# NorESMhub/BLOM

Hardware: AMD Instinct MI355X
Metric: simulated-days/sec (higher is better)
Workload: dtype f64; 1 GPU; channel 208x512x53 as 1 tile(s) of 208x512x53 along i, 1 tile per GPU, isopyc_bulkml/remap/geopotential/uc/enscon, ntr=3 (TKE, length-scale slot, ideal age: the reference default build), baclin=900s batrop=18s lstep=50; config 2's step (phy/mod_blom_step.F90:96-253: init_fluxes, tmsmt1, cmnfld2, difest_isobml [the whole routine: diffusivities estimated every step (NorESM defaults incl. rhsctp; the; physics=full, forcing=default, spinup_steps=0

## Files before the change

blom_amd/csrc/api.hip:

```cpp
#include "../../include/blomgpu.h"
#include "blomgpu_internal.h"
#include "pow_libm.h"
#include "sin_libm.h"
#include "atan2_libm.h"
#include <algorithm>
#include <cstring>
#include <string_view>

static thread_local std::string g_err;

int ctx_fail(blomgpu_ctx *c, const std::string &msg) {
  if (c) c->err = msg;
  g_err = msg;
  return 1;
}

void ctx_drop_graphs(blomgpu_ctx *c) {
  for (auto &g : c->step_graph)
    if (g) { (void)hipGraphExecDestroy(g); g = nullptr; }
  c->steps_warm = 0;
}

void ctx_sync_view(blomgpu_ctx *c) {
  if (!c->dirty) return;
// ... 401 lines not shown
  if (c->bt_flags) (void)hipFree(c->bt_flags);
  ale_free(c);
  dia_free(c);
  cesm_free(c);
  ben02_free(c);
  stepend_free(c);
  budget_free(c);
  if (c->ale_plevel) (void)hipFree(c->ale_plevel);
  if (c->arc_strip) (void)hipFree(c->arc_strip);
  if (c->xcsum_buf) (void)hipFree(c->xcsum_buf);
  if (c->xstream) (void)hipStreamDestroy(c->xstream);
  if (c->ev_fork) (void)hipEventDestroy(c->ev_fork);
  if (c->ev_join) (void)hipEventDestroy(c->ev_join);
  if (!c->stream_borrowed) (void)hipStreamDestroy(c->stream);
  delete c;
  return 0;
}

int blomgpu_sync(blomgpu_ctx *c) {
  HIPCHK(c, hipStreamSynchronize(c->stream));
  if (c->side) HIPCHK(c, hipStreamSynchronize(c->side));
  return 0;
}

int blomgpu_set_real(blomgpu_ctx *c, const char *name, double v) { return set_number(c, "blomgpu_set_real", name, 1u << O_REAL, v); }
int blomgpu_set_int(blomgpu_ctx *c, const char *name, int v) { return set_number(c, "blomgpu_set_int", name, 1u << O_INT | 1u << O_BOOL, v); }

int blomgpu_set_str(blomgpu_ctx *c, const char *name, const char *val) {
  const Opt *o = nullptr;
  const int rc = opt_lookup(c, "blomgpu_set_str", name, 1u << O_STR, &o);
  if (c) c->dirty = true;
  if (rc) return rc;
  if (!val) return ctx_fail(c, "blomgpu_set_str: null argument");
  const std::string v(val);
  if (!o->words[0].word) { *o->at(c).s = v; return 0; }
  for (const auto &w : o->words)
    if (w.word && v == w.word) {
      if (o->at) o->at(c).put(w.code);
      if (o->at && o->at(c).i == &c->swamth) c->swa_ready = false;
      return o->flags & ALE_RESET ? ale_reset(c) : 0;
    }
  return ctx_fail(c, o->refuse + v + " is unsupported!");
}

int blomgpu_get_real(blomgpu_ctx *c, const char *name, double *v) {
  const std::string s(name);
  if (const Opt *o = find_opt(s, 1u << O_REAL))
    if (o->flags & READABLE) { *v = *o->at(c).d; return 0; }
  if (s == "barotp_block_mode") { *v = bt_block_mode(c); return 0; }
  if (s == "barotp_shape") { *v = bt_shape_code(c); return 0; }
  if (s == "graph_steps") { *v = c->graph_steps; return 0; }
  if (s == "graph_failures") { *v = c->graph_failures; return 0; }
  if (s == "flux_diag_steps_skipped") { *v = (double)c->flux_diag_skipped; return 0; }
  if (s == "thermf_cesm_launches") { *v = (double)c->cesm_launches; return 0; }
  if (s == "thermf_ben02_launches") { *v = c->ben02_declared ? (double)c->cesm_launches : 0.; return 0; }
  if (c->step_time) {
    if (s == "xmi") { *v = c->xmi; return 0; }
    if (s == "nday_of_year") { *v = c->nday_of_year; return 0; }
    if (s.size() == 4 && s[0] == 'l' && s[1] >= '1' && s[1] <= '5' && s.compare(2, 2, "mi") == 0) { *v = c->lmi[s[1] - '1']; return 0; }
  }
  if (s == "sflxc") {
    if (!frc_declared(c)) return ctx_fail(c, "blomgpu_get_real: sflxc exists once blomgpu_inifrc_cesm has been called");
    double sum = 0.;
    HIPCHK(c, hipMemcpyAsync(&sum, c->cesm_sums, sizeof(double), hipMemcpyDeviceToHost, c->stream));
    HIPCHK(c, hipStreamSynchronize(c->stream));
    *v = sum / c->area;
    return 0;
  }
  if (s == "mxlayr_maxitr_entrain" || s == "mxlayr_maxitr_detrain") {
    *v = 0.;
    if (!c->err_dev) return 0;
    const int w = s == "mxlayr_maxitr_detrain" ? 5 : 6;
    int n = 0;
    HIPCHK(c, hipStreamSynchronize(c->stream));
    HIPCHK(c, hipMemcpy(&n, c->err_dev + w, sizeof(int), hipMemcpyDeviceToHost));
    HIPCHK(c, hipMemset(c->err_dev + w, 0, sizeof(int)));
    *v = n;
    return 0;
  }
  return ctx_fail(c, "blomgpu_get_real: unknown option " + s);
}

int blomgpu_option_name(int index, char *buf, int cap, int *kind) {
  if (index < 0 || index >= (int)(sizeof(g_opts) / sizeof(g_opts[0])) || !buf || cap < 2) return 1;
  snprintf(buf, cap, "%s", g_opts[index].name);
  if (kind) *kind = g_opts[index].kind;
  return 0;
}

int blomgpu_field_info(blomgpu_ctx *c, const char *name, int *nlev, int *is_int) {
  auto it = c->real_ids.find(name);
  if (it != c->real_ids.end()) {
    *nlev = ctx_real_nlev(c, it->second);
    if (std::string(name) == "trc" || std::string(name) == "trcold")
      *nlev = c->h.ntr * (std::string(name) == "trc" ? 2 : 1) * c->h.kk;
    *is_int = 0;
    return 0;
  }
  auto jt = c->int_ids.find(name);
  if (jt != c->int_ids.end()) { *nlev = c->nlev_int[jt->second]; *is_int = 1; return 0; }
  return ctx_fail(c, std::string("unknown field ") + name);
}

static int real_levels(blomgpu_ctx *c, const char *who, const char *name, int lev0, int nlev, double **ptr) {
  if (!c || !name) return ctx_fail(c, std::string(who) + ": null argument");
  auto it = c->real_ids.find(name);
// ... 472 lines not shown
    leave.failed = false;
  }
  if (!ale && (c->cmnfld1 || c->full_physics))
    if (int rc = stage(S_cmnfld1)) return rc;
  if (dia_active(c))
    if (int rc = st_diaacc(ALL6)) return rc;
  if (c->sprfac)
    if (int rc = st_fwbbal(c)) return rc;
  if (int rc = st_budget_output_instep(c)) return rc;
  if (c->chkvar) {
    c->seq.defer_checks = true;
    const int rc = st_chkvar(c, nn);
    c->seq.defer_checks = false;
    return rc;
  }
  return 0;
}
#undef ALL6
#undef STAGE_ARGS

int blomgpu_step(blomgpu_ctx *c, int *nstep, int nsteps) {
  const int kk = c->h.kk;
  if (int rc = dia_step_check(c)) return rc;
  if (cesm_on(c) && c->use_graph)
    return ctx_fail(c, "blomgpu_step: the coupled experiment's per-step scalars are kernel arguments, which a captured graph would freeze (set use_graph = 0)");
  if (ben02_on(c) && c->use_graph)
    return ctx_fail(c, "blomgpu_step: the forced ocean-ice experiment's per-step scalars are kernel arguments, which a captured graph would freeze (set use_graph = 0)");
  if (int rc = stepend_step_check(c)) return rc;
  const int ns0 = *nstep;
  if (int rc = budget_call_begin(c, ns0, nsteps)) return rc;
  struct FluxDiagBack { blomgpu_ctx *c; ~FluxDiagBack() { c->flux_diag = true; } } flux_diag_back{c};
  const bool flux_diag_lazy = !c->keep_flux_diag && c->h.P.vcoord_tag == 1 && !dia_reads_flux_diag(c);
  for (int it = 0; it < nsteps; it++) {
    const int ns = *nstep;
    const int m = ns % 2 + 1, n = (ns + 1) % 2 + 1;
    const int mm = (m - 1) * kk, nn = (n - 1) * kk, k1m = 1 + mm, k1n = 1 + nn;
    c->h.P.nstep = ns + 1;
    if (c->step_time)
      if (int rc = stepend_step_time(c, ns + 1)) return rc;
    ctx_sync_view(c);
    budget_call_slot(c, it);
    c->tmsmt1_ahead = !c->use_graph && !c->csdiag && it < nsteps - 1 && c->tmsmt_ahead && !dia_reads_dpold(c);
    c->flux_diag = !(flux_diag_lazy && !c->use_graph && !c->csdiag && it < nsteps - 2);
    bool graph = c->use_graph && !c->timing && !c->tiling.multi() && c->steps_warm >= 2 && !budget_on(c);
    hipGraphExec_t &ge = c->step_graph[ns & 1];
    if (graph && !ge) {
      bool began = false;
      auto capture = [&](hipGraphExec_t &out, int m_, int n_, int nstep_) {
        hipGraph_t g = nullptr;
        if (hipStreamBeginCapture(c->stream, hipStreamCaptureModeThreadLocal) != hipSuccess) return false;
        began = true;
        c->h.P.nstep = nstep_;
        const int mm_ = (m_ - 1) * kk, nn_ = (n_ - 1) * kk;
        const int rc = step_sequence(c, m_, n_, mm_, nn_, 1 + mm_, 1 + nn_);
        const hipError_t e = hipStreamEndCapture(c->stream, &g);
        bool ok = rc == 0 && e == hipSuccess && g != nullptr;
        if (ok && hipGraphInstantiate(&out, g, nullptr, nullptr, 0) != hipSuccess) { out = nullptr; ok = false; }
        if (g) (void)hipGraphDestroy(g);
        return ok;
      };
      bool ok = capture(ge, m, n, ns + 1);
      hipGraphExec_t &ge2 = c->step_graph[(ns + 1) & 1];
      if (ok && !ge2 && !capture(ge2, n, m, ns + 2)) ge2 = nullptr;
      c->h.P.nstep = ns + 1;
      if (!ok) {
        (void)hipGetLastError();
        c->err.clear();
        if (!began || ++c->graph_failures >= 3) c->use_graph = 0;
        else c->steps_warm = 0;
        graph = false;
      }
    }
    if (graph) { HIPCHK(c, hipGraphLaunch(ge, c->stream)); c->graph_steps++; }
    else if (int rc = step_sequence(c, m, n, mm, nn, k1m, k1n)) { c->tmsmt1_done_ahead = false; return rc; }
    if (!c->flux_diag) c->flux_diag_skipped++;
    dia_count(c);
    c->steps_done++;
    c->steps_warm++;
    const int period = (c->csdiag || c->timing) ? 1 : c->check_period;
    if (it == nsteps - 1)
      if (int rc = budget_call_fetch(c)) return rc;
    if (it == nsteps - 1 || (it + 1) % period == 0)
      if (int rc = ctx_check_errors(c)) {
        const int first = ns + 1 - (it % period);
        c->err += " (raised in one of the steps nstep = " + std::to_string(first) + ".." + std::to_string(ns + 1) + ")";
        c->tmsmt1_done_ahead = false;
        return rc;
      }
    const double delt2 = c->h.P.baclin + c->h.P.baclin;
    if (c->h.P.delt1 != delt2) { c->h.P.delt1 = delt2; c->dirty = true; }
    *nstep = ns + 1;
  }
  return budget_call_commit(c, ns0);
}

int blomgpu_dbg_bt_prof(blomgpu_ctx *c, long long *host, int nwords) {
  if (!host) {
    if (c->bt_prof) (void)hipFree(c->bt_prof);
    HIPCHK(c, hipMalloc((void **)&c->bt_prof, sizeof(long long) * nwords));
    HIPCHK(c, hipMemset(c->bt_prof, 0, sizeof(long long) * nwords));
    return 0;
  }
  HIPCHK(c, hipStreamSynchronize(c->stream));
  HIPCHK(c, hipMemcpy(host, c->bt_prof, sizeof(long long) * nwords, hipMemcpyDeviceToHost));
  return 0;
}

int blomgpu_dbg_kprof(blomgpu_ctx *c, long long *host, int nwords) {
  if (!host) {
    if (c->kprof) (void)hipFree(c->kprof);
    c->kprof = nullptr; c->kprof_words = 0;
    if (nwords <= 0) return 0;
    HIPCHK(c, hipMalloc((void **)&c->kprof, sizeof(long long) * nwords));
    HIPCHK(c, hipMemset(c->kprof, 0, sizeof(long long) * nwords));
    c->kprof_words = nwords;
    return 0;
  }
  if (!c->kprof || nwords > c->kprof_words) return ctx_fail(c, "blomgpu_dbg_kprof: no buffer of that size");
  HIPCHK(c, hipStreamSynchronize(c->stream));
  HIPCHK(c, hipMemcpy(host, c->kprof, sizeof(long long) * nwords, hipMemcpyDeviceToHost));
  return 0;
}

int blomgpu_timer_reset(blomgpu_ctx *c) {
  HIPCHK(c, hipStreamSynchronize(c->stream));
  for (auto &kv : c->timers) {
// ... 25 lines not shown
```

blom_amd/csrc/blomgpu_internal.h:

```cpp
#pragma once
#include <hip/hip_runtime.h>
#include <cstdint>
#include <string>
#include <unordered_map>
#include <vector>
#include "exp_libm.h"
#include "constants.h"
#include "workspace_slots.h"

#define NBDY 4

#ifdef BLOM_HOSTEMU
#define WAIT_VMCNT0() ((void)0)
#else
#define WAIT_VMCNT0() asm volatile("s_waitcnt vmcnt(0)" ::: "memory")
#endif

#define BLOM_REAL_FIELDS(X)                                                              \
                                                                          \
  X(u, 2 * K) X(v, 2 * K) X(dp, 2 * K) X(dpu, 2 * K) X(dpv, 2 * K) X(temp, 2 * K)        \
  X(saln, 2 * K) X(sigma, 2 * K) X(uflx, 2 * K) X(vflx, 2 * K) X(utflx, 2 * K)           \
  X(vtflx, 2 * K) X(usflx, 2 * K) X(vsflx, 2 * K)                                        \
  X(p, K + 1) X(pu, K + 1) X(pv, K + 1) X(phi, K + 1) X(cau, K) X(cav, K)                \
  X(ubflxs, 3) X(vbflxs, 3) X(ub, 2) X(vb, 2) X(pb, 2) X(pbu, 2) X(pbv, 2)               \
// ... 186 lines not shown
#define KPROF_MARK(wave, slot) do { if (kprof && 8 * (wave) + (slot) < kprof_words) kprof[8 * (wave) + (slot)] = wall_clock64(); } while (0)
#define KPROF_ADD(wave, slot, v) do { if (kprof && 8 * (wave) + (slot) < kprof_words) atomicAdd((unsigned long long *)&kprof[8 * (wave) + (slot)], (unsigned long long)(v)); } while (0)
#define KPROF_TRIP(wave, slot) do { if (kprof && 8 * (wave) + (slot) < kprof_words && (int)(threadIdx.x & 63) == __ffsll((long long)__ballot(1)) - 1) kprof[8 * (wave) + (slot)] += 1; } while (0)
#else
#define KPROF_ARGS
#define KPROF_PASS(id)
#define KPROF_MARK(wave, slot) do { } while (0)
#define KPROF_ADD(wave, slot, v) do { } while (0)
#define KPROF_TRIP(wave, slot) do { } while (0)
#endif

struct KTimer {
  double ms = 0.0;
  int launches = 0;
  std::vector<std::pair<hipEvent_t, hipEvent_t>> pending;
};

struct blomgpu_ctx;
struct TileGroup;
struct RcclComm;
struct BtGlobal;
struct DiaState;
struct BudgetState;
struct TileTable {
  int npx = 0, npy = 0, itdm = 0, nranks = 0;
  std::vector<int> i0, ii;
  std::vector<int> j0, jj;
  std::vector<int> rank;
  void ew_neighbours(int px, int py, bool periodic, int *west, int *east) const;
  bool tensor_product() const;
};
const char *tiletable_build(int npx, int npy, int itdm, int jtdm, const int *i0_pe, const int *ii_pe, const int *j0_pe,
                            const int *jj_pe, TileTable *out);
struct Tiling {
  int npx = 1, npy = 1;
  int px = 0, py = 0;
  const TileTable *tab = nullptr;
  TileGroup *group = nullptr;
  RcclComm *rccl = nullptr;
  bool multi() const { return npx * npy > 1 || rccl != nullptr; }
};

struct StepState {
  bool in_sequence = false;
  bool defer_checks = false;
  bool remap_handed_over = false;
  bool pbcor1_handed_over = false;
  bool pbcor2_handed_over = false;
  bool pbcor2_dp_in_wk = false;
  bool fluxes_lean = false;
  bool fluxes_zeroed = false;
  bool mom_early_done = false;
  bool convec_col_ahead = false;
  bool cmn_on_side = false;
  bool diapfl_mom_on_side = false, updtrc_on_side = false;
  bool pscan_done_ahead = false;
};

struct blomgpu_ctx {
  std::string expcnf = "channel";
  bool csdiag = false;
  int cnsvdi = 0;
  int cppm_compat = 1;
  int cppm_limiting = 2;
  int ale_method = 102, ale_upper_bndr_ord = 6, ale_lower_bndr_ord = 4, ale_tracer_limiting = 203, ale_velocity_limiting = 203;
  bool ale_tracer_pc_upper = true, ale_tracer_pc_lower = false, ale_velocity_pc_upper = true, ale_velocity_pc_lower = false;
  bool ale_density_pc_upper = false, ale_density_pc_lower = false;
  int ale_regrid_method = 2, ale_k_range_plevel = 1;
  double ale_regrid_nudge_ts = 86400., ale_stab_fac_limit = .75, ale_dpvar_fac = .75, ale_smooth_diff_max = 50000.;
  int ale_dktzu = 4, ale_dktzl = 2;
  double ale_dpmin_interior = .1 * ONEM;
  int ndiff_rec_per_face = 0;
  int ndiff_surface_align = 1;
  double rm0 = 1.2, rm5 = 0., niwgf = 0., niwbf = .35, niwlf = .5;
  std::string mlrttp = "constant";
  double trxday = 0., srxday = 0., trxdpt = 1., srxdpt = 1., trxlim = 1.5, srxlim = .5, sref = 34.65, area = 0., xmi = 0.;
  int lmi[5] = {11, 12, 1, 2, 3};
  bool aptflx = false, apsflx = false, ditflx = false, disflx = false, srxbal = false;
  int ntda = 0;
  double swamxd = 200., brine_mlbase_frac = 0.;
  int mlrmth = 1;
  double eddtra_ce = .06, tau_mlr = 86400., tau_growing_hbl = 300., tau_decaying_hbl = 86400., tau_growing_hml = 3600.,
         tau_decaying_hml = 259200., lfmin = 5.e3, mlbl_max_ratio = 3., eddtra_cl = .25, mstar = .5, nstar = .066, wpup_min = 1.e-3;
  double egc = 0., eggam = 200., eglsmn = 4000., egmndf = 0., egmxdf = 1500., egidfq = 1., rhiscf = 0., ri0 = 1.2, tkepf = 0.;
  double bdml_logc = 0.;
  int eddf2d = 0, edsprs = 1, edanis = 0, redi3d = 0, rhsctp = 0, edfsmo = 0;
  int edritp_opt = 2, edwmth_opt = 1;
  bool smtfrc = false, use_stream_relaxation = false;
  int nstep_in_cpl = 1, l1ci = 1, l2ci = 1, nstep_in_day = 1, nday_of_year = 1;
  int cesm_single_sums = 0;
  bool full_physics = false;
  int difest_live = 0;
  int live_slopes = 0;
  int cmnfld1 = 0;
  int eddtra_frozen = 0;
  int check_period = 8;
  bool timing = false;
  int use_graph = 0;
  int overlap = 1;
  int phys_dag = 7;
  int mom_early_at = 0;
  int lean_fluxes = 1;
  int tmsmt_fold = 1;
  int tmsmt_ahead = 1;
  int remap_fold = 0;
  int remap_nfirst = 4;
  int halo_overlap = 1;
  int barotp_fused = 1;
  int barotp_tile = 0;
  int barotp_persist = 1;
  int barotp_block = 1;
  int barotp_overlap = 0;
  int barotp_rimbuf = 1;
  int barotp_arctic_persist = 1;
  int barotp_arctic_fused = 1;
  int arctic_strips = 0;
  int pgf_uv_pair = 0;
  int pgf_uv_ring = 7;
  int pgf_reuse = 0;
  int pgf_copy_fused = 1;
  int scan_reassoc = 0;
  int mom_aw_split = 0;
  int mom_force_aw = 0;
  int momtum_order = 0;
  int momtum_lds_pad = 0;
  int momtum_bs = 0;
  int momtum_chunks_a = 0, momtum_chunks_b = 0;
  int convec_nsingle = 2;
  int cmn_nslope_nb = 4;
  int diapfl_du = 8;
  int diffus_shfl = 0;
  int kprof_sel = 1;

  DevView h;
  DevView *d = nullptr;
  bool dirty = true;
  int device = 0;
  hipStream_t stream = nullptr;
  bool stream_borrowed = false;
  hipStream_t xstream = nullptr, halo_stream = nullptr;
  hipEvent_t ev_fork = nullptr, ev_join = nullptr;
  hipStream_t side = nullptr;
  hipEvent_t ev_side[10] = {};
  DevView hv[4];
  DevView *dv[4] = {nullptr, nullptr, nullptr, nullptr};
  double *wk_mom = nullptr, *p_alt = nullptr, *pu_alt = nullptr, *pv_alt = nullptr;
  hipStream_t side3 = nullptr;
  hipEvent_t ev_side3[2] = {nullptr, nullptr};
  int mom_aw_key = -1, mom_aw_n[2] = {0, 0};
  int *mom_aw_dev = nullptr;
  int nlev_real[NF_REAL];
  int nlev_int[NF_INT];
  std::unordered_map<std::string, int> real_ids, int_ids;
  std::unordered_map<std::string, KTimer> timers;
  Tiling tiling;
  BtGlobal *bt_global = nullptr;
  std::string err;
  int *err_dev = nullptr;
  StepState seq;
  bool tmsmt1_ahead = false, tmsmt1_done_ahead = false;
  bool flux_diag = true, keep_flux_diag = false;
  long long flux_diag_skipped = 0;
  hipGraphExec_t step_graph[2] = {nullptr, nullptr};
  int steps_done = 0;
  int steps_warm = 0;
  long long graph_steps = 0;
  int graph_failures = 0;
  bool cppm_ready = false;
  void *ale = nullptr;
  double *ale_plevel = nullptr;
  bool bt_restart = true;
  unsigned bt_epoch = 0;
  unsigned *bt_flags = nullptr;
  int bt_flags_words = 0;
  int num_cus = 0;
  int bt4_blocks_per_cu[2] = {-1, -1};
  int bt_blocks_per_cu[4] = {-1, -1, -1, -1};
  long long *bt_prof = nullptr;
  long long *kprof = nullptr;
  int kprof_words = 0;
  double *arc_strip = nullptr;
  size_t arc_cap = 0;
  double *xcsum_dev = nullptr;
  double *xcsum_buf = nullptr;
  double budget[5][7][2] = {};
  int budget_step = 0;
  BudgetState *bud = nullptr;
  DiaState *dia = nullptr;
  std::vector<double> dia_edges;
  std::vector<double> dia_sigdia;
  bool cesm_declared = false;
  int nflxdi[48] = {};
  long long cesm_launches = 0;
  double *cesm_sums = nullptr, *cesm_rows = nullptr;
  bool ben02_declared = false;
  double *ben02_planes = nullptr;
  bool step_time = false;
  int swamth = 0;
  int jwtype = 0;
  std::string chlopt = "climatology";
  bool swa_ready = false;
  double *swa_lut = nullptr;
  double swa_log10chl_min = 0., swa_dlog10chl = 0.;
  bool sprfac = false;
  double prfac = 1.;
  bool chkvar = false;
  double *fwb_buf = nullptr;
  unsigned long long *chk_dev = nullptr;
  int dia_alarm = -1;
};
enum { VIEW_MAIN = 0, VIEW_MOM_A, VIEW_MOM_B, VIEW_MOM_C, NVIEW };
static inline const DevView *ctx_view(const blomgpu_ctx *c, int which) { return which == VIEW_MAIN ? c->d : c->dv[which]; }
int ctx_side_fork(blomgpu_ctx *c, int ev);
int ctx_side_done(blomgpu_ctx *c, int ev);
// ... 56 lines not shown
int ben02_reset_tda(blomgpu_ctx *);
void ben02_free(blomgpu_ctx *);
int st_sfcstr_ben02(blomgpu_ctx *);
int st_thermf_ben02(blomgpu_ctx *, int m, int n, int mm, int nn, int k1m, int k1n);
enum { SWA_NONE = 0, SWA_TOP_LAYER, SWA_JERLOV, SWA_MA94, SWA_OHL03, SWA_SPATIAL };
static inline bool swa_chlorophyll(const blomgpu_ctx *c) { return c->swamth == SWA_MA94 || c->swamth == SWA_OHL03; }
int stepend_iniswa(blomgpu_ctx *);
int stepend_set_sprfac(blomgpu_ctx *);
int stepend_step_time(blomgpu_ctx *, int ns1);
int stepend_step_check(blomgpu_ctx *);
int stepend_check_errors(blomgpu_ctx *);
void stepend_free(blomgpu_ctx *);
int st_updswa(blomgpu_ctx *);
int st_fwbbal(blomgpu_ctx *);
int st_chkvar(blomgpu_ctx *, int nn);
static inline double *ctx_real_ptr(const blomgpu_ctx *c, int id) {
  if (id < FID_BEN02) return c->h.f[id];
  if (id >= FID_STEPEND) return c->h.e[id - FID_STEPEND];
  return c->ben02_planes ? c->ben02_planes + (size_t)(id - FID_BEN02) * c->h.nplane : nullptr;
}
static inline int ctx_real_nlev(const blomgpu_ctx *c, int id) { return id < FID_BEN02 ? c->nlev_real[id] : id >= FID_STEPEND ? kStepEndLevels[id - FID_STEPEND] : 1; }
int st_xcsum_batch(blomgpu_ctx *, int nb, const double *const *planes, const int *const *masks, double *rows, double *out);
int st_niw_ke_tendency(blomgpu_ctx *, int m, int mm);
int st_difest_isobml_pre(blomgpu_ctx *, int m, int n, int mm, int nn);
int st_difest_isobml(blomgpu_ctx *, int m, int n, int mm, int nn);
static inline bool budget_on(const blomgpu_ctx *c) { return c->budget_step && c->cnsvdi; }
int st_budget_sums(blomgpu_ctx *, int ncall, int n, int nn);
int st_budget_init(blomgpu_ctx *);
int st_budget_output(blomgpu_ctx *, int m);
int st_budget_instep(blomgpu_ctx *, int ncall, int off);
int st_budget_output_instep(blomgpu_ctx *);
int budget_call_begin(blomgpu_ctx *, int ns, int nsteps);
void budget_call_slot(blomgpu_ctx *, int it);
int budget_call_fetch(blomgpu_ctx *);
int budget_call_commit(blomgpu_ctx *, int ns);
int budget_steps(blomgpu_ctx *, int *first, int *count);
int budget_mass0(blomgpu_ctx *, double *mass0);
int budget_record(blomgpu_ctx *, int nstep, double *rec);
int budget_line(blomgpu_ctx *, int nstep, int file, double *terms, int *nterms);
int budget_files(blomgpu_ctx *, int *mask);
void budget_free(blomgpu_ctx *);
int st_barotp(blomgpu_ctx *, int m, int n, int mm, int nn, int k1m, int k1n);
int st_eddtra(blomgpu_ctx *, int m, int n, int mm, int nn, int k1m, int k1n);
int st_eddtra_ale(blomgpu_ctx *, int m, int n, int mm, int nn, int k1m, int k1n);
int st_cppm(blomgpu_ctx *, int m, int n, int mm, int nn, int k1m, int k1n);
int st_init_cppm(blomgpu_ctx *);
int st_mxlayr_tail(blomgpu_ctx *, int nn, int k1n);
int ctx_err_words(blomgpu_ctx *);
int ctx_check_errors(blomgpu_ctx *);
int st_kfpla_halo(blomgpu_ctx *, int n);
int st_cmnfld1(blomgpu_ctx *, int m, int n, int mm, int nn, int k1m, int k1n);
int st_cmnfld2(blomgpu_ctx *, int m, int n, int mm, int nn, int k1m, int k1n);
int diapfl_column3_launch(blomgpu_ctx *, int n, int nn, int *errflag);
int st_ale_vdifft(blomgpu_ctx *, int m, int n, int mm, int nn, int k1m, int k1n);
int st_ale_vdiffm(blomgpu_ctx *, int m, int n, int mm, int nn, int k1m, int k1n);
int st_ale_forcing(blomgpu_ctx *, int m, int n, int mm, int nn, int k1m, int k1n);
int st_cmnfld_bfsqi_ale(blomgpu_ctx *, int m, int n, int mm, int nn, int k1m, int k1n);
int st_ale_regrid_remap(blomgpu_ctx *, int m, int n, int mm, int nn, int k1m, int k1n);
int st_ale_remap_diazlv(blomgpu_ctx *, int m, int n, int mm, int nn, int k1m, int k1n);
void ale_free(blomgpu_ctx *);
int ale_check_deferred(blomgpu_ctx *);
int st_mxlayr(blomgpu_ctx *, int m, int n, int mm, int nn, int k1m, int k1n);
int st_diaacc(blomgpu_ctx *, int m, int n, int mm, int nn, int k1m, int k1n);
int dia_select(blomgpu_ctx *, const char *names);
int dia_reset(blomgpu_ctx *);
int dia_finalize(blomgpu_ctx *);
int dia_nacc(blomgpu_ctx *, int *nacc);
int dia_get(blomgpu_ctx *, const char *name, double *out);
int dia_name(int index, char *buf, int cap, int *is_lyr, int *grid);
int dia_name_all(int index, char *buf, int cap, int *kind, int *grid);
int dia_name_full(int index, char *buf, int cap, int *kind, int *grid);
int dia_name_ext(int index, char *buf, int cap, int *kind, int *grid);
bool dia_reads_mldl82(const blomgpu_ctx *);
bool dia_reads_dpold(const blomgpu_ctx *);
bool dia_reads_flux_diag(const blomgpu_ctx *);
double *dia_acc_span(const blomgpu_ctx *, size_t *n);
int dia_set_sigdia(blomgpu_ctx *, const double *sigdia, int n);
int dia_get_sigdia(blomgpu_ctx *, double *out, int cap, int *n);
int dia_set_levels(blomgpu_ctx *, const double *bnds, int ddm);
int dia_levels_levitus2x(blomgpu_ctx *);
int dia_get_levels(blomgpu_ctx *, double *bnds, int cap, int *ddm);
int dia_alarm(blomgpu_ctx *, int alarm);
struct DiaHyb { int ddm; double *acc; const double *edges; int temp, saln, uvel, vvel; };
bool dia_hybrid_slots(const blomgpu_ctx *, DiaHyb *);
int dia_step_check(blomgpu_ctx *);
bool dia_active(const blomgpu_ctx *);
void dia_count(blomgpu_ctx *);
void dia_free(blomgpu_ctx *);
int st_mom_pupv(blomgpu_ctx *, int off, int lo, int hi);
int st_convec_velocity(blomgpu_ctx *, int nn);
int launch_dpudpv(blomgpu_ctx *, int off, int flags);
int launch_p_dpu_dpv(blomgpu_ctx *, int off, int flags);
int remap_tile_launch(blomgpu_ctx *, int n, int mm, int nn, int tsel, bool fold);
int pbcor_tile_launch(blomgpu_ctx *, int which, int m, int offc, int offf, int from_remap);
int launch_pscan(blomgpu_ctx *, int off, int lo, int hi_off);
int st_xctilr(blomgpu_ctx *, double *base, int l1, int ld, int mh, int nh, int itype);
int st_xctilr_arctic_multi(blomgpu_ctx *, int nf, double *const *ptrs, const int *nlevs, const int *mhs, const int *nhs,
                           const int *itypes);
int st_xctilr_multi(blomgpu_ctx *, int nf, double *const *ptrs, const int *nlevs, int mh, int nh, const int *itypes);
int st_crc(blomgpu_ctx *, const double *base, int nlev, int itype, unsigned *crc);
int st_crc_strips(blomgpu_ctx *, double *base, int nlev, int itype, unsigned *out, int cap, int *l0, int *ns);
int ctx_locate_ptr(const blomgpu_ctx *, const double *p, size_t *offset);
int rccl_xctilr(blomgpu_ctx *, double *base, int nlev, int mhl, int nhl);
int rccl_barotp_replicated(blomgpu_ctx *, int m, int n, int mm, int nn, int k1m, int k1n);
blomgpu_ctx *bt_global_ctx(const blomgpu_ctx *);
struct RcclLanded {
// ... 71 lines not shown
```

blom_amd/csrc/stage_diapfl.hip:

```cpp
#include "blomgpu_internal.h"
#include "eos.h"

#define AR(slot, k) WK(V, slot)[c + (size_t)((k)-1) * np]

#include "diapfl_common.h"

__global__ void k_diapfl_kming(const DevView *__restrict__ Vp) {
  const DevView &V = *Vp;
  THREAD_IJ_XCD(V);
  if (j < 0 || j > V.jj + 1 || i < 0 || i > V.ii + 1 || !V.m[I_ip][c]) return;
  V.m[I_kming][c] = (int)rint(V.f[F_util1][c]);
}


__device__ inline void diapfl_mom_flux_v(double pm, double fum, double flm, double pc, double fuc, double flc, double pzb,
                                         double &fpu_k, double &fpl_km1) {
  double fpum, fplm, fpup, fplp;
  double pnew = pm, fu = fum, fl = flm;
  double pold = pnew - fl + fu;
  if (pold <= pzb) {
    if (pnew <= pzb) { fpum = fu; fplm = fl; } else { fpum = fu; fplm = fl - pnew + pzb; }
  } else {
    if (pnew <= pzb) { fpum = fu - pold + pzb; fplm = fl; } else { fpum = .5 * (fu + fl); fplm = fpum; }
  }
// ... 99 lines not shown
      const int lq = kq == kmin ? 1 : (kq == kmin + 1 ? 2 : kq);
      b0[u] = LV(vel, lq); b1[u] = AR(sb + U_GTD, kq);
    }
#pragma unroll
    for (int u = 0; u < 2 * MU_; u++) {
      const int k = k0 - u;
      if (k < kmin) break;
      const int lay = k == kmin ? 1 : (k == kmin + 1 ? 2 : k);
      unext = b0[u] - gnext * unext;
      LV(vel, lay) = unext;
      gnext = b1[u];
    }
  }
  const double ub = uprev;
  for (int k0 = kmax + 1; k0 <= kk; k0 += 2 * MU_) {
    double b0[2 * MU_], b1[2 * MU_];
#pragma unroll
    for (int u = 0; u < 2 * MU_; u++) {
      const int kq = k0 + u <= kk ? k0 + u : kk;
      b0[u] = p[mns + (size_t)(kq - 1) * np]; b1[u] = LV(p, kq);
    }
#pragma unroll
    for (int u = 0; u < 2 * MU_; u++)
      if (k0 + u <= kk && fmin2(b0[u], b1[u]) < pzb) LV(vel, k0 + u) = ub;
  }
}

__global__ void k_diapfl_dpudpv(const DevView *__restrict__ Vp, int nn) {
  const DevView &V = *Vp;
  THREAD_IJ_XCD(V);
  const int k = by_;
  const size_t np = V.nplane, o0 = (size_t)k * np, o1 = (size_t)(k + 1) * np, ob = (size_t)V.kk * np;
  gcd_t p = V.f[F_p];
  if (V.m[I_iu][c] && j >= 1 && j <= V.jj && i >= 1 && i <= V.ii + 1) {
    const size_t w = c - 1;
    const double q = fmin2(p[c + ob], p[w + ob]);
    V.f[F_dpu][c + (size_t)(k + nn) * np] = .5 * ((fmin2(q, p[w + o1]) - fmin2(q, p[w + o0])) + (fmin2(q, p[c + o1]) - fmin2(q, p[c + o0])));
  }
  if (V.m[I_iv][c] && j >= 1 && j <= V.jj + 1 && i >= 1 && i <= V.ii) {
    const size_t s = c - V.ni;
    const double q = fmin2(p[c + ob], p[s + ob]);
    V.f[F_dpv][c + (size_t)(k + nn) * np] = .5 * ((fmin2(q, p[s + o1]) - fmin2(q, p[s + o0])) + (fmin2(q, p[c + o1]) - fmin2(q, p[c + o0])));
  }
}

int st_diapfl(blomgpu_ctx *c, int n, int nn, int k1n) {
  (void)k1n;
  const DevView &h = c->h;
  if (h.P.vcoord_tag != 1) return ctx_fail(c, "diapfl is only called for isopyc_bulkml (phy/mod_blom_step.F90:172-186)");
  if (int rc = ctx_err_words(c)) return rc;
  int *errflag = c->err_dev + 0;
  {
    TimeScope ts(c, "diapfl");
    if (int rc = diapfl_column3_launch(c, n, nn, errflag)) return rc;
    {
      double *ptrs[4] = {h.f[F_p], h.f[F_fpug], h.f[F_fplg], h.f[F_util1]};
      const int nl[4] = {h.kk + 1, h.kk, h.kk, 1}, it[4] = {1, 1, 1, 1};
      if (int rc = st_xctilr_multi(c, 4, ptrs, nl, 1, 1, it)) return rc;
    }
    hipLaunchKernelGGL(k_diapfl_kming, plane_grid(h), dim3(256), 0, c->stream, c->d);
    const bool aside = ctx_overlap_on(c) && (c->phys_dag & 2) && !c->tiling.multi() && c->full_physics;
    hipStream_t s = c->stream;
    if (aside) {
      if (int rc = ctx_side_fork(c, 6)) return rc;
      s = c->side;
    }
    hipLaunchKernelGGL(k_diapfl_momentum, plane_grid(h, 2, 64), dim3(64), 0, s, c->d, nn);
    if (!c->seq.in_sequence || c->full_physics) hipLaunchKernelGGL(k_diapfl_dpudpv, plane_grid(h, h.kk), dim3(256), 0, s, c->d, nn);
    if (aside) {
      if (int rc = ctx_side_done(c, 7)) return rc;
      c->seq.diapfl_mom_on_side = true;
    }
  }
  HIPCHK(c, hipGetLastError());
  if (!c->seq.defer_checks) return ctx_check_errors(c);
  return 0;
}
```

blom_amd/csrc/stage_diapfl_col3.hip:

```cpp
#include "diapfl_common.h"

#define MAXTR 4
#define CLAMPK(k, lo, hi) ((k) < (lo) ? (lo) : ((k) > (hi) ? (hi) : (k)))

#define WNS (D3_NSLOT + 1)
#define W(slot, k) wb[((size_t)((k)-1) * WNS + (slot)) * 64]
#define ST(a, k) (a)[c + (size_t)((k)-1) * np]
#define SIGR(k) sigr[c + (size_t)((k)-1) * np]
#define PRES(k) wb[((size_t)((k)-1) * WNS + D3_NSLOT) * 64]
#define TRC(nt, k) trc[c + (size_t)((k)-1 + (nt)*2 * kk) * np]

template <int DU>
__global__ void __launch_bounds__(64, 1) k_diapfl_column3(const DevView *__restrict__ Vp, int n, int nn, int *__restrict__ errflag KPROF_ARGS) {
  const DevView &V = *Vp;
  constexpr int DH = DU < 4 ? DU : 4;
  const int t_ = blockIdx.x * blockDim.x + threadIdx.x;
  if (t_ >= V.nplane) return;
  const int i = t_ % V.ni - (NBDY - 1), j = t_ / V.ni - (NBDY - 1);
  const size_t c = t_;
  if (j < 1 || j > V.jj || i < 1 || i > V.ii || !V.m[I_ip][c]) return;
  const size_t np = V.nplane;
  const int kk = V.kk, ntr = V.ntr;
  const Params P = V.P;
  const double dsgmnr = .1, fcmxr = .25, dsgcr0 = .25, dfeps = 1.e-12, gbbl = .2, kappa = .4, ustmin = .0001;
  const double cc = GRAV * GRAV * P.delt1 / (ALPHA0 * ALPHA0);
  [[maybe_unused]] const int wid = blockIdx.x;
  KPROF_MARK(wid, 0);
  gcd_t __restrict__ sigr = V.f[F_sigmar];
  gd_t __restrict__ wb = global_ptr(V.wk) + (size_t)blockIdx.x * (kk + 1) * WNS * 64 + threadIdx.x;
  gd_t __restrict__ temp = V.f[F_temp] + (size_t)nn * np, saln = V.f[F_saln] + (size_t)nn * np;
  gd_t __restrict__ dp = V.f[F_dp] + (size_t)nn * np, sigma = V.f[F_sigma] + (size_t)nn * np;
  gd_t __restrict__ trc = V.f[F_trc] + (size_t)nn * np, nu = V.f[F_difdia];
  gd_t __restrict__ fpug = V.f[F_fpug], fplg = V.f[F_fplg];

  int kmax = 1;
  for (int k0 = 2; k0 <= kk; k0 += 2 * DU) {
    double a0[2 * DU];
#pragma unroll
    for (int u = 0; u < 2 * DU; u++) a0[u] = ST(dp, CLAMPK(k0 + u, 2, kk));
#pragma unroll
    for (int u = 0; u < 2 * DU; u++)
      if (k0 + u <= kk && a0[u] > EPSILP) kmax = k0 + u;
  }
  const int kfpl = V.m[I_kfpla][c + (size_t)(n - 1) * np];
  const int kmin = kfpl - 2;
  double fpl0 = 0., fpl1 = 0.;
  const bool mixing = kmin < kmax;
  if (mixing) {
    const double d1 = ST(dp, 1), d2 = ST(dp, 2);
    double acc = 0.;
    acc = acc + d1;
    const double p1 = acc;
    acc = acc + d2;
    const double preskf = acc;
    PRES(kfpl) = acc;
    for (int k0 = kfpl; k0 <= kmax; k0 += 2 * DU) {
      double a0[2 * DU];
#pragma unroll
      for (int u = 0; u < 2 * DU; u++) a0[u] = ST(dp, CLAMPK(k0 + u, kfpl, kmax));
#pragma unroll
      for (int u = 0; u < 2 * DU; u++)
        if (k0 + u <= kmax) { acc = acc + a0[u]; PRES(k0 + u + 1) = acc; }
    }
    const double presb = acc;
    {
      fpl0 = fmin2(fmin2(p1, presb - p1), cc * ST(nu, 1) * (d1 + d2) / (2. * d1 * d2));
      const double delpu = fmax2(ONEM, d2), delpl = fmax2(ONEM, ST(dp, kfpl <= kk ? kfpl : kk));
      fpl1 = fmin2(fmin2(preskf, presb - preskf), cc * ST(nu, 2) * (delpu + delpl) / (2. * delpu * delpl));
      if (kmax == kmin + 1) fpl1 = 0.;
    }
    if (kfpl <= kmax) {
      int k;
      if (kfpl < kmax) {
        k = kmax - 1;
        const double us = V.f[F_ustarb][c];
        const double nubbl = gbbl * (us * us * us) *
                             exp_libm(-(ST(dp, k + 1) + .5 * ST(dp, k)) * fabs(V.f[F_coriop][c]) * ALPHA0 /
                                 (kappa * fmax2(ustmin, us) * GRAV)) /
                             (ALPHA0 * GRAV * (SIGR(k + 1) - SIGR(k)));
        ST(nu, k) = fmax2(ST(nu, k), nubbl);
      }
      const int rst1 = kfpl;
// ... 435 lines not shown
        const int k = k0 + u;
        if (k > kfpl - 1) break;
        ST(temp, k) = tf;
        ST(sigma, k) = a0[u];
        ST(saln, k) = eosd::sofsig(P, a0[u], tf);
        ST(dp, k) = 0.;
#pragma unroll
        for (int nt = 0; nt < MAXTR; nt++)
          if (nt < ntr) TRC(nt, k) = trf[nt];
      }
    }
    for (int nt = MAXTR; nt < ntr; nt++) {
      const double xf = TRC(nt, kfpl), xm = TRC(nt, kmax);
      for (int k = 3; k <= kfpl - 1; k++) TRC(nt, k) = xf;
      for (int k = kmax + 1; k <= kk; k++) TRC(nt, k) = xm;
    }
    for (int k0 = kmax + 1; k0 <= kk; k0 += 2 * DU) {
      double a0[2 * DU];
#pragma unroll
      for (int u = 0; u < 2 * DU; u++) a0[u] = SIGR(CLAMPK(k0 + u, kmax + 1, kk));
#pragma unroll
      for (int u = 0; u < 2 * DU; u++) {
        const int k = k0 + u;
        if (k > kk) break;
        ST(temp, k) = tm;
        ST(sigma, k) = a0[u];
        ST(saln, k) = eosd::sofsig(P, a0[u], tm);
#pragma unroll
        for (int nt = 0; nt < MAXTR; nt++)
          if (nt < ntr) TRC(nt, k) = trm[nt];
      }
    }
  }
  if (P.itrtke >= 1) {
    const int a = P.itrtke - 1, b = P.itrgls - 1;
    const bool doa = a < ntr, dob = P.gls && b >= 0 && b < ntr;
    for (int k0 = 1; k0 <= kk; k0 += 2 * DU) {
      double a0[2 * DU], a1[2 * DU];
#pragma unroll
      for (int u = 0; u < 2 * DU; u++) {
        const int kq = CLAMPK(k0 + u, 1, kk);
        a0[u] = doa ? TRC(a, kq) : 0.;
        a1[u] = dob ? TRC(b, kq) : 0.;
      }
#pragma unroll
      for (int u = 0; u < 2 * DU; u++) {
        const int k = k0 + u;
        if (k > kk) break;
        if (doa) TRC(a, k) = fmax2(a0[u], TKE_MIN);
        if (dob) TRC(b, k) = fmax2(a1[u], GLS_PSI_MIN);
      }
    }
  }
  column_scan(V.f[F_p][c], dp + c, V.f[F_p] + c, np, kk);
  V.f[F_util1][c] = (double)kmin;
  if (mixing) {
    for (int k = 1; k <= kmin; k++) { ST(fpug, k) = fpl0; ST(fplg, k) = fpl0; }
    ST(fpug, kmin + 1) = fpl0;
    ST(fplg, kmin + 1) = fpl1;
    for (int k = kmax + 1; k <= kk; k++) { ST(fpug, k) = 0.; ST(fplg, k) = 0.; }
  } else
    for (int k = 1; k <= kk; k++) { ST(fpug, k) = 0.; ST(fplg, k) = 0.; }
  KPROF_MARK(wid, 5);
}

int diapfl_column3_launch(blomgpu_ctx *c, int n, int nn, int *errflag) {
  const DevView &h = c->h;
  if (D3_NSLOT > h.nwk) return ctx_fail(c, "diapfl: work space too small");
  const dim3 g = plane_grid(h, 1, 64);
  if ((size_t)g.x * (h.kk + 1) * WNS * 64 > (size_t)h.nwk * h.kk * h.nplane) return ctx_fail(c, "diapfl: work space too small");
  TimeScope tk(c, "k_diapfl_column3");
  if (c->diapfl_du == 8) hipLaunchKernelGGL(k_diapfl_column3<8>, g, dim3(64), 0, c->stream, c->d, n, nn, errflag KPROF_PASS(2));
  else if (c->diapfl_du == 2) hipLaunchKernelGGL(k_diapfl_column3<2>, g, dim3(64), 0, c->stream, c->d, n, nn, errflag KPROF_PASS(2));
  else hipLaunchKernelGGL(k_diapfl_column3<4>, g, dim3(64), 0, c->stream, c->d, n, nn, errflag KPROF_PASS(2));
  return 0;
}
```

blom_amd/csrc/stage_momtum.hip:

```cpp
#include "blomgpu_internal.h"

#include "momtum_common.h"


__global__ void k_mom_pupv(const DevView *__restrict__ Vp, int off, int lo, int hi, int ring) {
  const DevView &V = *Vp;
  THREAD_IJ_XCD(V);
  if (j < lo || j > V.jj + hi || i < lo || i > V.ii + hi) return;
  if (ring && j >= 1 && j <= V.jj && i >= 1 && i <= V.ii) return;
  const size_t np = V.nplane;
  if (V.m[I_iu][c]) column_scan(V.f[F_pu][c], V.f[F_dpu] + (size_t)off * np + c, V.f[F_pu] + c, np, V.kk);
  if (V.m[I_iv][c]) column_scan(V.f[F_pv][c], V.f[F_dpv] + (size_t)off * np + c, V.f[F_pv] + c, np, V.kk);
}

__global__ void k_mom_pscan(const DevView *__restrict__ Vp, int off, int lo, int hi, int ring) {
  const DevView &V = *Vp;
  THREAD_IJ_XCD(V);
  if (j < lo || j > V.jj + hi || i < lo || i > V.ii + hi || !V.m[I_ip][c]) return;
  if (ring && j >= 1 && j <= V.jj && i >= 1 && i <= V.ii) return;
  const size_t np = V.nplane;
  column_scan(V.f[F_p][c], V.f[F_dp] + (size_t)off * np + c, V.f[F_p] + c, np, V.kk);
}

__global__ void k_mom_drag(const DevView *__restrict__ Vp, int n, int nn) {
// ... 34 lines not shown
  const double tsfac = V.P.dlt / V.P.delt1;
  gd_t q = WK2(V, S2_QUM);
  if (V.m[I_iu][c]) {
    const double sy = V.f[F_scuy][c];
    q[c] = V.f[F_ubflxs_p][c + om] * tsfac / (V.f[F_pbu][c + om] * sy);
    q[c + 2 * np] = V.f[F_ubflxs_p][c + on] * tsfac / (V.f[F_pbu][c + on] * sy);
  }
  if (V.m[I_iv][c]) {
    const double sx = V.f[F_scvx][c];
    q[c + np] = V.f[F_vbflxs_p][c + om] * tsfac / (V.f[F_pbv][c + om] * sx);
    q[c + 3 * np] = V.f[F_vbflxs_p][c + on] * tsfac / (V.f[F_pbv][c + on] * sx);
  }
}

int st_mom_pupv(blomgpu_ctx *c, int off, int lo, int hi) {
  hipLaunchKernelGGL(k_mom_pupv, plane_grid(c->h, 1, 64), dim3(64), 0, c->stream, c->d, off, lo, hi, 0);
  HIPCHK(c, hipGetLastError());
  return 0;
}

static int momtum_visc_chain(blomgpu_ctx *c, int m, int n, int mm, int nn) {
  const DevView &h = c->h;
  hipLaunchKernelGGL(k_mom_pupv, plane_grid(h, 1, 64), dim3(64), 0, c->stream, ctx_view(c, VIEW_MOM_A), mm, -1, 2, 0);
  hipLaunchKernelGGL(k_mom_qplanes, plane_grid(h, 1, 256), dim3(256), 0, c->stream, ctx_view(c, VIEW_MOM_A), m, n);
  return st_momtum_fused_layers(c, m, n, mm, nn, 1);
}

int st_momtum_early(blomgpu_ctx *c, int m, int n, int mm, int nn) {
  c->seq.mom_early_done = false;
  if (!ctx_overlap_on(c) || c->tiling.multi()) return 0;
  if (int rc = st_xctilr(c, c->h.f[F_difwgt], 1, 1, 2, 2, 1)) return rc;
  if (int rc = ctx_side_fork(c, 0)) return rc;
  hipStream_t main = c->stream;
  c->stream = c->side;
  const int rc = momtum_visc_chain(c, m, n, mm, nn);
  c->stream = main;
  if (rc) return rc;
  if (int rc2 = ctx_side_done(c, 1)) return rc2;
  c->seq.mom_early_done = true;
  return 0;
}

int st_momtum(blomgpu_ctx *c, int m, int n, int mm, int nn, int k1m, int k1n) {
  (void)k1m; (void)k1n;
  const DevView &h = c->h;
  const dim3 gcol = plane_grid(h, 1, 64), b64(64);
  if (ctx_overlap_on(c) && !c->tiling.multi())
    if (int rc = st_convec_column_ahead(c, n, nn)) return rc;
  TimeScope ts(c, "momtum");
  hipLaunchKernelGGL(k_mom_pscan, gcol, b64, 0, c->stream, ctx_view(c, VIEW_MOM_B), mm, -1, 2, 0);
  hipLaunchKernelGGL(k_mom_pscan, gcol, b64, 0, c->stream, c->d, mm, -1, 2, c->seq.in_sequence && h.P.vcoord_tag == 1 ? 1 : 0);
  hipLaunchKernelGGL(k_mom_pupv, gcol, b64, 0, c->stream, c->d, mm, -1, 2, 1);
  hipLaunchKernelGGL(k_mom_drag, gcol, b64, 0, c->stream, ctx_view(c, VIEW_MOM_B), n, nn);
  if (c->seq.mom_early_done) {
    c->seq.mom_early_done = false;
    if (int rc = ctx_side_join(c, 1)) return rc;
  } else {
    if (int rc = st_xctilr(c, h.f[F_difwgt], 1, 1, 2, 2, 1)) return rc;
    if (int rc = momtum_visc_chain(c, m, n, mm, nn)) return rc;
  }
  return st_momtum_fused_layers(c, m, n, mm, nn, 2);
}
```

blom_amd/csrc/workspace_slots.h:

```cpp
#pragma once

#define NWK2D 48
enum Wk2dSlot {
  S2_PBFACO = 0, S2_REMAP_PM = S2_PBFACO, S2_PBFACN = 1, S2_PBUT = S2_PBFACN, S2_PBVT = 2, S2_DRAG = 3, S2_QUM = 4, S2_VRTSFL = 8,
  S2_PBFACM = 9, S2_BVFBOT = 10, S2_EXPB = 11, S2_NEXT_FREE = 12
};
static_assert(S2_QUM + 4 == S2_VRTSFL && S2_NEXT_FREE <= NWK2D, "momtum's four planes end in front of thermf's; the planes fit");

constexpr int wk_slots(int ntr) { return 32 + 5 * (ntr > 0 ? ntr : 1); }

enum { CP_HM = 0, CP_HF, CP_HPC0, CP_HPC1, CP_HPC2, CP_TE };
#define CP_HTF(ntl) (CP_TE + (ntl))
#define CP_TPC0(ntl) (CP_TE + 2 * (ntl))
#define CP_TPC1(ntl) (CP_TE + 3 * (ntl))
#define CP_TPC2(ntl) (CP_TE + 4 * (ntl))
#define CP_NSLOT(ntl) (CP_TE + 5 * (ntl))

enum { RG_DX = 0, RG_DY, RG_TX, RG_TY, RG_TD, RG_SX, RG_SY, RG_SD };
#define RG_TRX(nt) (8 + 3 * (nt))
#define RG_TRY(nt) (9 + 3 * (nt))
#define RG_TRD(nt) (10 + 3 * (nt))
#define F_BASE(ntr) (8 + 3 * (ntr))
#define RF_DU(ntr) (F_BASE(ntr) + 0)
#define RF_DV(ntr) (F_BASE(ntr) + 1)
#define RF_TU(ntr) (F_BASE(ntr) + 2)
#define RF_TV(ntr) (F_BASE(ntr) + 3)
#define RF_SU(ntr) (F_BASE(ntr) + 4)
#define RF_SV(ntr) (F_BASE(ntr) + 5)
#define RF_TRU(ntr, nt) (F_BASE(ntr) + 6 + 2 * (nt))
#define RF_TRV(ntr, nt) (F_BASE(ntr) + 7 + 2 * (nt))
#define R_BASE(ntr) (8 + 3 * (ntr))
#define R_DP(ntr) (R_BASE(ntr) + 0)
#define R_T(ntr) (R_BASE(ntr) + 1)
#define R_S(ntr) (R_BASE(ntr) + 2)
#define R_TR(ntr, nt) (R_BASE(ntr) + 3 + (nt))
static_assert(F_BASE(3) == R_BASE(3) && F_BASE(0) == R_BASE(0), "R_DP.. reuse the flux planes' slots");

enum { N_DP = 0, N_S = 1, N_T = 2 };
#define N_TR(nt) (3 + (nt))
static_assert(R_BASE(0) > N_TR(0) - 1 && R_BASE(64) > N_TR(64 - 1), "remap's hand-over lies behind pbcor's new state");

enum { DF_DU2 = 0, DF_DV2, DF_BVFSQ, DF_BVF, DF_EGR, DF_ANISOK, DF_SM1, DF_SM2, DF_NUB, DF_NSLOT };

enum { CM_DELP = 0, CM_BFSQ, CM_SLS2, CM_GAM_ALE, CM_GAM = DF_NSLOT, CM_NSLOT };
static_assert(CM_GAM >= DF_NSLOT, "cmnfld2 beside difest_isobml: no common slot");

enum { ED_MFL = 0, ED_SPARE, ED_DLM, ED_DLP, ED_NSLOT };
enum { EA_PUV = 0, EA_GM, EA_SM, EA_MFL, EA_DLM, EA_DLP, EA_NARR };
enum { U_GTD = 0, U_NSLOT };
enum { D3_SU = 0, D3_SL, D3_FCU, D3_FCL, D3_FMAX, D3_H, D3_R, D3_T, D3_F, D3_FT, D3_GTD, D3_NSLOT };
enum { CV_UN = 0 };
enum { DH_POT = 0, DH_POTPB, DH_A, DH_T, DH_ALPR, DH_NSLOT };
enum { VD_GAM0 = 0, VD_GAM1 };
enum { MF_VISU = 0, MF_VISV, MF_UM, MF_UN, MF_VM, MF_VN, MF_NSLOT };

constexpr int wk_need_cppm(int ntr) { return CP_NSLOT(2 + ntr); }
constexpr int wk_need_remap(int ntr) { return ntr > 0 ? RF_TRV(ntr, ntr - 1) + 1 : RF_SV(ntr) + 1; }
constexpr int wk_need_handover(int ntr) { return R_TR(ntr, ntr); }
constexpr int wk_need_pbcor(int ntr) { return N_TR(ntr); }
constexpr int wk_max(int a, int b) { return a > b ? a : b; }
constexpr int wk_need_fixed() {
  return wk_max(wk_max(wk_max(DF_NSLOT, CM_NSLOT), wk_max(2 * ED_NSLOT, 2 * EA_NARR + 3)),
                wk_max(wk_max(2 * U_NSLOT, D3_NSLOT), wk_max(wk_max(CV_UN + 2, DH_NSLOT), VD_GAM1 + 1)));
}
constexpr bool wk_fits(int ntr) {
  return wk_need_cppm(ntr) <= wk_slots(ntr) && wk_need_remap(ntr) <= wk_slots(ntr) && wk_need_handover(ntr) <= wk_slots(ntr) &&
         wk_need_pbcor(ntr) <= wk_slots(ntr) && wk_need_fixed() <= wk_slots(ntr);
}
static_assert(wk_fits(0) && wk_fits(1) && wk_fits(3) && wk_fits(24) && wk_fits(64), "a stage's slots do not fit into wk_slots(ntr)");
```

Measured before the change: 1.692 simulated-days/sec.

## Run diapfl column kernel ahead on side stream during momtum

Launches the diapycnal-flux column kernel early on the side stream, right after momtum's drag kernel, when convec's column work and early momentum are already forked. The main stream joins later in diapfl, and a small finish kernel does the pressure column scan and writes kmin into util1. This is meant to hide the serial column kernel behind momtum work. It enables the path by default via phys_dag bit 16, shifts the kernel's workspace to a separate slot base, adds a 2D kmin slot, and counts ahead steps, including under graph replay. Running concurrently with other kernels risks contention for compute units.

```diff
diff --git a/blom_amd/csrc/api.hip b/blom_amd/csrc/api.hip
--- a/blom_amd/csrc/api.hip
+++ b/blom_amd/csrc/api.hip
@@ -477,6 +477,7 @@
   if (s == "graph_steps") { *v = c->graph_steps; return 0; }
   if (s == "graph_failures") { *v = c->graph_failures; return 0; }
   if (s == "flux_diag_steps_skipped") { *v = (double)c->flux_diag_skipped; return 0; }
+  if (s == "diapfl_ahead_steps") { *v = (double)c->diapfl_ahead_steps; return 0; }
   if (s == "thermf_cesm_launches") { *v = (double)c->cesm_launches; return 0; }
   if (s == "thermf_ben02_launches") { *v = c->ben02_declared ? (double)c->cesm_launches : 0.; return 0; }
   if (c->step_time) {
@@ -1055,7 +1056,10 @@
         began = true;
         c->h.P.nstep = nstep_;
         const int mm_ = (m_ - 1) * kk, nn_ = (n_ - 1) * kk;
+        const long long ahead0 = c->diapfl_ahead_steps;
         const int rc = step_sequence(c, m_, n_, mm_, nn_, 1 + mm_, 1 + nn_);
+        c->graph_diapfl_ahead[(nstep_ - 1) & 1] = (int)(c->diapfl_ahead_steps - ahead0);
+        c->diapfl_ahead_steps = ahead0;
         const hipError_t e = hipStreamEndCapture(c->stream, &g);
         bool ok = rc == 0 && e == hipSuccess && g != nullptr;
         if (ok && hipGraphInstantiate(&out, g, nullptr, nullptr, 0) != hipSuccess) { out = nullptr; ok = false; }
@@ -1074,7 +1078,7 @@
         graph = false;
       }
     }
-    if (graph) { HIPCHK(c, hipGraphLaunch(ge, c->stream)); c->graph_steps++; }
+    if (graph) { HIPCHK(c, hipGraphLaunch(ge, c->stream)); c->graph_steps++; c->diapfl_ahead_steps += c->graph_diapfl_ahead[ns & 1]; }
     else if (int rc = step_sequence(c, m, n, mm, nn, k1m, k1n)) { c->tmsmt1_done_ahead = false; return rc; }
     if (!c->flux_diag) c->flux_diag_skipped++;
     dia_count(c);
diff --git a/blom_amd/csrc/blomgpu_internal.h b/blom_amd/csrc/blomgpu_internal.h
--- a/blom_amd/csrc/blomgpu_internal.h
+++ b/blom_amd/csrc/blomgpu_internal.h
@@ -262,6 +262,7 @@
   bool fluxes_zeroed = false;
   bool mom_early_done = false;
   bool convec_col_ahead = false;
+  bool diapfl_col_ahead = false;
   bool cmn_on_side = false;
   bool diapfl_mom_on_side = false, updtrc_on_side = false;
   bool pscan_done_ahead = false;
@@ -308,7 +309,7 @@
   bool timing = false;
   int use_graph = 0;
   int overlap = 1;
-  int phys_dag = 7;
+  int phys_dag = 23;
   int mom_early_at = 0;
   int lean_fluxes = 1;
   int tmsmt_fold = 1;
@@ -351,7 +352,7 @@
   hipStream_t xstream = nullptr, halo_stream = nullptr;
   hipEvent_t ev_fork = nullptr, ev_join = nullptr;
   hipStream_t side = nullptr;
-  hipEvent_t ev_side[10] = {};
+  hipEvent_t ev_side[12] = {};
   DevView hv[4];
   DevView *dv[4] = {nullptr, nullptr, nullptr, nullptr};
   double *wk_mom = nullptr, *p_alt = nullptr, *pu_alt = nullptr, *pv_alt = nullptr;
@@ -370,6 +371,8 @@
   StepState seq;
   bool tmsmt1_ahead = false, tmsmt1_done_ahead = false;
   bool flux_diag = true, keep_flux_diag = false;
+  long long diapfl_ahead_steps = 0;
+  int graph_diapfl_ahead[2] = {0, 0};
   long long flux_diag_skipped = 0;
   hipGraphExec_t step_graph[2] = {nullptr, nullptr};
   int steps_done = 0;
@@ -532,6 +535,8 @@
 int st_cmnfld1(blomgpu_ctx *, int m, int n, int mm, int nn, int k1m, int k1n);
 int st_cmnfld2(blomgpu_ctx *, int m, int n, int mm, int nn, int k1m, int k1n);
 int diapfl_column3_launch(blomgpu_ctx *, int n, int nn, int *errflag);
+int st_diapfl_column_ahead(blomgpu_ctx *, int n, int nn);
+int st_diapfl_column_join(blomgpu_ctx *, int nn);
 int st_ale_vdifft(blomgpu_ctx *, int m, int n, int mm, int nn, int k1m, int k1n);
 int st_ale_vdiffm(blomgpu_ctx *, int m, int n, int mm, int nn, int k1m, int k1n);
 int st_ale_forcing(blomgpu_ctx *, int m, int n, int mm, int nn, int k1m, int k1n);
diff --git a/blom_amd/csrc/stage_diapfl.hip b/blom_amd/csrc/stage_diapfl.hip
--- a/blom_amd/csrc/stage_diapfl.hip
+++ b/blom_amd/csrc/stage_diapfl.hip
@@ -175,7 +175,9 @@
   int *errflag = c->err_dev + 0;
   {
     TimeScope ts(c, "diapfl");
-    if (int rc = diapfl_column3_launch(c, n, nn, errflag)) return rc;
+    if (c->seq.diapfl_col_ahead) {
+      if (int rc = st_diapfl_column_join(c, nn)) return rc;
+    } else if (int rc = diapfl_column3_launch(c, n, nn, errflag)) return rc;
     {
       double *ptrs[4] = {h.f[F_p], h.f[F_fpug], h.f[F_fplg], h.f[F_util1]};
       const int nl[4] = {h.kk + 1, h.kk, h.kk, 1}, it[4] = {1, 1, 1, 1};
diff --git a/blom_amd/csrc/stage_diapfl_col3.hip b/blom_amd/csrc/stage_diapfl_col3.hip
--- a/blom_amd/csrc/stage_diapfl_col3.hip
+++ b/blom_amd/csrc/stage_diapfl_col3.hip
@@ -10,7 +10,7 @@
 #define PRES(k) wb[((size_t)((k)-1) * WNS + D3_NSLOT) * 64]
 #define TRC(nt, k) trc[c + (size_t)((k)-1 + (nt)*2 * kk) * np]
 
-template <int DU>
+template <int DU, bool AHEAD>
 __global__ void __launch_bounds__(64, 1) k_diapfl_column3(const DevView *__restrict__ Vp, int n, int nn, int *__restrict__ errflag KPROF_ARGS) {
   const DevView &V = *Vp;
   constexpr int DH = DU < 4 ? DU : 4;
@@ -27,7 +27,7 @@
   [[maybe_unused]] const int wid = blockIdx.x;
   KPROF_MARK(wid, 0);
   gcd_t __restrict__ sigr = V.f[F_sigmar];
-  gd_t __restrict__ wb = global_ptr(V.wk) + (size_t)blockIdx.x * (kk + 1) * WNS * 64 + threadIdx.x;
+  gd_t __restrict__ wb = WK(V, AHEAD ? D3_BASE_AHEAD : D3_BASE) + (size_t)blockIdx.x * (kk + 1) * WNS * 64 + threadIdx.x;
   gd_t __restrict__ temp = V.f[F_temp] + (size_t)nn * np, saln = V.f[F_saln] + (size_t)nn * np;
   gd_t __restrict__ dp = V.f[F_dp] + (size_t)nn * np, sigma = V.f[F_sigma] + (size_t)nn * np;
   gd_t __restrict__ trc = V.f[F_trc] + (size_t)nn * np, nu = V.f[F_difdia];
@@ -569,8 +569,12 @@
       }
     }
   }
-  column_scan(V.f[F_p][c], dp + c, V.f[F_p] + c, np, kk);
-  V.f[F_util1][c] = (double)kmin;
+  if constexpr (AHEAD) {
+    WK2(V, S2_KMIN)[c] = (double)kmin;
+  } else {
+    column_scan(V.f[F_p][c], dp + c, V.f[F_p] + c, np, kk);
+    V.f[F_util1][c] = (double)kmin;
+  }
   if (mixing) {
     for (int k = 1; k <= kmin; k++) { ST(fpug, k) = fpl0; ST(fplg, k) = fpl0; }
     ST(fpug, kmin + 1) = fpl0;
@@ -581,14 +585,55 @@
   KPROF_MARK(wid, 5);
 }
 
-int diapfl_column3_launch(blomgpu_ctx *c, int n, int nn, int *errflag) {
+__global__ void __launch_bounds__(64) k_diapfl_ahead_finish(const DevView *__restrict__ Vp, int nn) {
+  const DevView &V = *Vp;
+  THREAD_IJ_XCD(V);
+  if (j < 1 || j > V.jj || i < 1 || i > V.ii || !V.m[I_ip][c]) return;
+  const size_t np = V.nplane;
+  column_scan(V.f[F_p][c], V.f[F_dp] + (size_t)nn * np + c, V.f[F_p] + c, np, V.kk);
+  V.f[F_util1][c] = WK2(V, S2_KMIN)[c];
+}
+
+static int diapfl_column3_launch_on(blomgpu_ctx *c, hipStream_t s, bool ahead, int n, int nn, int *errflag) {
   const DevView &h = c->h;
-  if (D3_NSLOT > h.nwk) return ctx_fail(c, "diapfl: work space too small");
+  const int base = ahead ? D3_BASE_AHEAD : D3_BASE;
+  if (base + D3_NSLOT > h.nwk) return ctx_fail(c, "diapfl: work space too small");
   const dim3 g = plane_grid(h, 1, 64);
-  if ((size_t)g.x * (h.kk + 1) * WNS * 64 > (size_t)h.nwk * h.kk * h.nplane) return ctx_fail(c, "diapfl: work space too small");
-  TimeScope tk(c, "k_diapfl_column3");
-  if (c->diapfl_du == 8) hipLaunchKernelGGL(k_diapfl_column3<8>, g, dim3(64), 0, c->stream, c->d, n, nn, errflag KPROF_PASS(2));
-  else if (c->diapfl_du == 2) hipLaunchKernelGGL(k_diapfl_column3<2>, g, dim3(64), 0, c->stream, c->d, n, nn, errflag KPROF_PASS(2));
-  else hipLaunchKernelGGL(k_diapfl_column3<4>, g, dim3(64), 0, c->stream, c->d, n, nn, errflag KPROF_PASS(2));
+  if ((size_t)base * h.kk * h.nplane + (size_t)g.x * (h.kk + 1) * WNS * 64 > (size_t)h.nwk * h.kk * h.nplane) return ctx_fail(c, "diapfl: work space too small");
+  TimeScope tk(c, "k_diapfl_column3", s);
+#define D3_LAUNCH(DU)                                                                                                         \
+  do {                                                                                                                        \
+    if (ahead) hipLaunchKernelGGL((k_diapfl_column3<DU, true>), g, dim3(64), 0, s, c->d, n, nn, errflag KPROF_PASS(2));       \
+    else hipLaunchKernelGGL((k_diapfl_column3<DU, false>), g, dim3(64), 0, s, c->d, n, nn, errflag KPROF_PASS(2));            \
+  } while (0)
+  if (c->diapfl_du == 8) D3_LAUNCH(8);
+  else if (c->diapfl_du == 2) D3_LAUNCH(2);
+  else D3_LAUNCH(4);
+#undef D3_LAUNCH
   return 0;
 }
+
+int diapfl_column3_launch(blomgpu_ctx *c, int n, int nn, int *errflag) { return diapfl_column3_launch_on(c, c->stream, false, n, nn, errflag); }
+
+int st_diapfl_column_ahead(blomgpu_ctx *c, int n, int nn) {
+  const DevView &h = c->h;
+  c->seq.diapfl_col_ahead = false;
+  if (!(c->phys_dag & 16) || !c->seq.in_sequence || !ctx_overlap_on(c) || c->tiling.multi() || h.P.vcoord_tag != 1 || h.ntr > MAXTR ||
+      budget_on(c) || !c->seq.convec_col_ahead || !c->seq.mom_early_done)
+    return 0;
+  if (int rc = ctx_err_words(c)) return rc;
+  if (int rc = ctx_side_fork(c, 10)) return rc;
+  if (int rc = diapfl_column3_launch_on(c, c->side, true, n, nn, c->err_dev + 0)) return rc;
+  HIPCHK(c, hipGetLastError());
+  if (int rc = ctx_side_done(c, 11)) return rc;
+  c->seq.diapfl_col_ahead = true;
+  c->diapfl_ahead_steps++;
+  return 0;
+}
+
+int st_diapfl_column_join(blomgpu_ctx *c, int nn) {
+  c->seq.diapfl_col_ahead = false;
+  if (int rc = ctx_side_join(c, 11)) return rc;
+  hipLaunchKernelGGL(k_diapfl_ahead_finish, plane_grid(c->h, 1, 64), dim3(64), 0, c->stream, c->d, nn);
+  return 0;
+}
diff --git a/blom_amd/csrc/stage_momtum.hip b/blom_amd/csrc/stage_momtum.hip
--- a/blom_amd/csrc/stage_momtum.hip
+++ b/blom_amd/csrc/stage_momtum.hip
@@ -110,6 +110,7 @@
   hipLaunchKernelGGL(k_mom_pscan, gcol, b64, 0, c->stream, c->d, mm, -1, 2, c->seq.in_sequence && h.P.vcoord_tag == 1 ? 1 : 0);
   hipLaunchKernelGGL(k_mom_pupv, gcol, b64, 0, c->stream, c->d, mm, -1, 2, 1);
   hipLaunchKernelGGL(k_mom_drag, gcol, b64, 0, c->stream, ctx_view(c, VIEW_MOM_B), n, nn);
+  if (int rc = st_diapfl_column_ahead(c, n, nn)) return rc;
   if (c->seq.mom_early_done) {
     c->seq.mom_early_done = false;
     if (int rc = ctx_side_join(c, 1)) return rc;
diff --git a/blom_amd/csrc/workspace_slots.h b/blom_amd/csrc/workspace_slots.h
--- a/blom_amd/csrc/workspace_slots.h
+++ b/blom_amd/csrc/workspace_slots.h
@@ -3,7 +3,7 @@
 #define NWK2D 48
 enum Wk2dSlot {
   S2_PBFACO = 0, S2_REMAP_PM = S2_PBFACO, S2_PBFACN = 1, S2_PBUT = S2_PBFACN, S2_PBVT = 2, S2_DRAG = 3, S2_QUM = 4, S2_VRTSFL = 8,
-  S2_PBFACM = 9, S2_BVFBOT = 10, S2_EXPB = 11, S2_NEXT_FREE = 12
+  S2_PBFACM = 9, S2_BVFBOT = 10, S2_EXPB = 11, S2_KMIN = 12, S2_NEXT_FREE = 13
 };
 static_assert(S2_QUM + 4 == S2_VRTSFL && S2_NEXT_FREE <= NWK2D, "momtum's four planes end in front of thermf's; the planes fit");
 
@@ -50,6 +50,8 @@
 enum { U_GTD = 0, U_NSLOT };
 enum { D3_SU = 0, D3_SL, D3_FCU, D3_FCL, D3_FMAX, D3_H, D3_R, D3_T, D3_F, D3_FT, D3_GTD, D3_NSLOT };
 enum { CV_UN = 0 };
+enum { D3_BASE = 0, D3_BASE_AHEAD = 2 };
+static_assert(D3_BASE_AHEAD >= CV_UN + 2, "diapfl's column kernel beside convec's velocity remap: no common slot");
 enum { DH_POT = 0, DH_POTPB, DH_A, DH_T, DH_ALPR, DH_NSLOT };
 enum { VD_GAM0 = 0, VD_GAM1 };
 enum { MF_VISU = 0, MF_VISV, MF_UM, MF_UN, MF_VM, MF_VN, MF_NSLOT };
```

Result: no change. 1.719 simulated-days/sec (median of 6 runs) (+1.6%).
